# WanqingXia/UR-gym

Hardware: AMD Instinct MI355X
Metric: env-steps/sec (whole node) (higher is better)
Workload: dtype f64; 1 GPU; UR5DynReach-v1 N=65536 per GPU, random actions U(-1,1), auto-reset, seed 0; envs_total=65536, gather_obs=False, rollout_api=False, gjk_start=bullet

## Files before the change

ur_gym_amd/csrc/urgym_hip.hip:

```cpp
#include <hip/hip_runtime.h>
#include <stdint.h>
#include <stdio.h>
#include <string.h>
#include <math.h>
#include <new>
#include <vector>

#include "../../include/urgym.h"
#include "../../data/ur5e_model.h"
#include "urgym_device.h"
#include "urgym_launch_plan.h"
#include "urgym_actor.h"
#include "urgym_tables_host.h"

using namespace urgym;


namespace {

constexpr int WAVES = 4;
constexpr int THREADS = GROUP * WAVES;
constexpr uint32_t NO_ITEM = 0xFFFFFFFFu;
constexpr int REFILL_MIN = 16;
constexpr int RESIDENT = 3;
// ... 416 lines not shown
  int& s_left = L.s_left;
  auto& s_key = L.s_key;
  auto& s_pose = L.s_pose;

  const urgym_config& cfg = P.cfg;
  const urgym_buffers& B = P.buf;
  const int N = cfg.num_envs;
  const int tid = threadIdx.x;
  const int lane = tid & 63;
  const int wv = __builtin_amdgcn_readfirstlane(tid >> 6);
  constexpr int OD = (KIND == URGYM_ENV_ORI) ? 18 : ((KIND == URGYM_ENV_OBS) ? 26 : ((KIND == URGYM_ENV_STA) ? 29 : 35));
  constexpr int GD = (KIND == URGYM_ENV_OBS) ? 3 : 6;
  int vb = bidx;
  if (MODE == MODE_STEP && P.envs_tail == 0) {
    const int nb = nblk, x = vb & 7, per = nb >> 3, rem = nb & 7;
    vb = x * per + (x < rem ? x : rem) + (vb >> 3);
  }
  const bool tail_block = (MODE == MODE_STEP) && P.envs_tail > 0 && vb >= P.big_blocks;
  const int E = tail_block ? P.envs_tail : P.envs;
  const int first = tail_block ? P.big_blocks * P.envs + (vb - P.big_blocks) * P.envs_tail : vb * P.envs;
  const int G = (E + GROUP - 1) / GROUP;
  constexpr bool HAS_OBST = (KIND != URGYM_ENV_ORI);
  constexpr int COLL_BIT = 1 << 30;
  constexpr int EE_BIT = 1 << 29;
  constexpr int EPA_SHIFT = 8, EPA_MASK = 0x7FFF << EPA_SHIFT;
  const bool need_epa = WITH_EPA && ((KIND == URGYM_ENV_OBS) || !cfg.check_collision || (MODE != MODE_STEP));
  XRef pose_slot{(URGYM_LDS double*)&s_pose[0][0] + tid, THREADS};
  float* const s_out = reinterpret_cast<float*>(&s_pose[0][0]);
  static_assert(sizeof(float) * STEP_MAX_ENVS * 47 <= sizeof(double) * GJK_SLOT_DOUBLES * THREADS, "staging must fit");
  auto dist_cell = [&](int i, int e) -> double* {
    return DIST_LDS ? (double*)&s_dist[i][DIST_LDS ? e : 0] : &P.ld_scratch[(size_t)i * N + first + e];
  };

  if (bidx == 0 && tid == 0) {
    if (P.rzero) *P.rzero = 0;
    if (P.rzero2) *P.rzero2 = 0;
  }
  int list_count = 0;
  if (MODE != MODE_STEP) {
    list_count = (MODE == MODE_PREFETCH) ? min(*P.rcount, P.rcap) : B.done_count[P.pp];
    if (first >= list_count) return;
  }
  if (tid == 0) { s_ticket = THREADS; s_pending = 0; s_p1done = 0; s_left = 0; }
  if (MODE == MODE_STEP && tid < 8) {
    const int k = tid & 3, ex = tid >> 2;
    const bool tbl = (k == Q_TABLE);
    const double msum = M_HULL + ((k == 3) ? M_CYL : ((k == Q_SELF) ? M_HULL : (tbl ? M_TABLE : M_TRACK)));
// ... 85 lines not shown
      D3 a0[3], a1[3];
#pragma unroll
      for (int k = 0; k < 6; k++) {
        double sn, cs;
        if (use_cache) { sn = SOA(P.sc_scratch, 2 * k, n, N); cs = SOA(P.sc_scratch, 2 * k + 1, n, N); }
        else sincos(q[k], &sn, &cs);
        fk_joint(T, k, sn, cs);
        const int link = k + 1;
        const double* c = c_tab.capsule[k];
        const D3 b0 = apply(T, d3(c[0], c[1], c[2])), b1 = apply(T, d3(c[3], c[4], c[5]));
        const double rb = c[6];
        if (k < 3) { a0[k] = b0; a1[k] = b1; }
        if (link >= 2) {
          if (seg_box_lower_bound(b0, b1, TABLE_CX, TABLE_CY, TABLE_CZ, TABLE_HX, TABLE_HY, TABLE_HZ) - rb <= lim) pairs |= 1u << (PAIR_TABLE + link - 2);
          if (seg_box_lower_bound(b0, b1, TRACK_CX, TRACK_CY, TRACK_CZ, TRACK_HX, TRACK_HY, TRACK_HZ) - rb <= lim) pairs |= 1u << (PAIR_TRACK + link - 2);
        }
#pragma unroll
        for (int A = 1; A <= 3; A++) {
          if (A <= link - 2) {
            if (segseg_dist(a0[A - 1], a1[A - 1], b0, b1) - c_tab.capsule[A - 1][6] - rb <= lim + M_HULL) pairs |= 1u << self_pair_bit(A, link);
          }
        }
      }
      if (MODE == MODE_STEP) {
        double er, ep, ey;
        rpy_from_quat(rot_to_quat(T.r), er, ep, ey);
        float* orow = B.observation + (size_t)n * OD;
        orow[0] = (float)T.t.x; orow[1] = (float)T.t.y; orow[2] = (float)T.t.z;
        orow[3] = (float)er; orow[4] = (float)ep; orow[5] = (float)ey;
        atomicOr(&s_flags[e], EE_BIT);
      }
    }
    s_pairs[e] = pairs;
    if (pairs) atomicAdd(&s_pending, __popc(pairs));
  }
  if (MODE == MODE_STEP) {
    if (wv >= WAVES - G && lane == 0) __hip_atomic_fetch_add(&s_p1done, 1, __ATOMIC_RELEASE, __HIP_MEMORY_SCOPE_WORKGROUP);
  } else {
    __syncthreads();
  }

  if (!(MODE == MODE_STEP && !HAS_OBST && !cfg.check_collision)) {
    D3 v0 = d3(0, 1, 0);
    int kind = 3, e = 0, lb = 2, la = 1;
    auto shape_a = [&]() -> ShapeDesc { return hull_desc(kind == Q_SELF ? la : lb); };
    auto shape_b = [&]() -> ShapeDesc {
      ShapeDesc s;
      s.type = (kind == 3) ? SH_CYLZ : ((kind == Q_SELF) ? SH_HULL : SH_BOX);
      s.hull = lb - 1;
      const bool tbl = (kind == Q_TABLE);
      s.hx = (kind == 3) ? (CYL_R - M_CYL) : (tbl ? (TABLE_HX - M_TABLE) : (TRACK_HX - M_TRACK));
      s.hy = (kind == 3) ? (CYL_R - M_CYL) : (tbl ? (TABLE_HY - M_TABLE) : (TRACK_HY - M_TRACK));
      s.hz = (kind == 3) ? (0.5 * CYL_H - M_CYL) : (tbl ? (TABLE_HZ - M_TABLE) : (TRACK_HZ - M_TRACK));
      return s;
    };
    bool exact = false;
    const bool guided = cfg.gjk_start == URGYM_GJK_START_GUIDED;
    auto capsule_mid = [&](int link, const X3& TX) -> D3 {
      const double* c = c_tab.capsule[link - 1];
      return apply(TX, d3(0.5 * (c[0] + c[3]), 0.5 * (c[1] + c[4]), 0.5 * (c[2] + c[5])));
    };
    auto guided_axis = [&](D3 mid, D3 centre) -> D3 {
      const D3 d = mid - centre;
      const double n2 = dot(d, d);
      return n2 > 1e-12 ? d * (1.0 / sqrt(n2)) : d3(0, 1, 0);
// ... 126 lines not shown
      }
      typedef int pool_words __attribute__((ext_vector_type(4)));
      const pool_words pool = *(volatile URGYM_LDS pool_words*)(URGYM_LDS void*)&s_ticket;
      __builtin_amdgcn_fence(__ATOMIC_ACQUIRE, "workgroup");
      const bool more_tickets = pool.x < n_tickets;
      const bool p1_published = (MODE != MODE_STEP) || pool.z >= G;
      const bool more_pairs = pool.y > 0;
      if (MODE == MODE_STEP) p1_ok = p1_published;
      const int idle_lanes = __popcll(__ballot(!busy));
      if (!busy && (idle_lanes >= REFILL_MIN || idle_lanes == 64)) {
        uint32_t item = NO_ITEM;
        if (more_tickets) {
          const int t = atomicAdd(&s_ticket, 1);
          if (t < n_tickets) item = ticket_item(t);
        } else if (more_pairs) {
          if (atomicSub(&s_pending, 1) > 0) item = claim_pair();
        }
        if (item != NO_ITEM) {
          busy = setup(item);
          if (busy) gjk_begin(run, v0);
        }
      }
      if (__ballot(busy) == 0ull && !more_tickets && !more_pairs && p1_published) break;
    }
    auto epa_pass = [&]() -> bool {
      const EpaWs ws{(URGYM_LDS double*)&s_pose[0][0] + GROUP * wv, THREADS};
      bool armed = false;
#pragma unroll 1
      for (int g = 0; g < G; g++) {
        const int sl = g * GROUP + lane;
        const int marks = (sl < E) ? ((__hip_atomic_load(&s_flags[sl], __ATOMIC_RELAXED, __HIP_MEMORY_SCOPE_WORKGROUP) & EPA_MASK) >> EPA_SHIFT) : 0;
        unsigned long long envs_marked = __ballot(marks != 0);
#pragma unroll 1
        while (envs_marked) {
          const int el = __builtin_ctzll(envs_marked);
          envs_marked &= envs_marked - 1ull;
          const int ee = g * GROUP + el;
          int me = __shfl(marks, el);
#pragma unroll 1
          while (me) {
            const int b = __builtin_ctz((unsigned)me);
            me &= me - 1;
            int mine = 0;
            if (lane == 0) mine = (atomicAnd(&s_flags[ee], ~(1 << (EPA_SHIFT + b))) >> (EPA_SHIFT + b)) & 1;
            if (!__shfl(mine, 0)) continue;
            if (!armed) {
// ... 1 lines not shown
              if (MODE == MODE_STEP) p1_ok = true;
              armed = true;
            }
            const int body = b / 5, link = 2 + b - 5 * body;
            const uint32_t item = (uint32_t)ee | ((uint32_t)(body == 0 ? 3 : (body == 1 ? Q_TABLE : Q_TRACK)) << 8) | ((uint32_t)link << 10) |
                                  ((body ? 1u : 0u) << 16);
            if (!setup(item)) continue;
            epa_wave_sync();
            bool capped;
            const double depth = epa_wave(P.graph, shape_a(), shape_b(), ws, lane, capped);
            if (lane == 0) {
              const double dist = -(depth + margin_sum());
              if (workbench) atomicMin(reinterpret_cast<long long*>(dist_cell(lb - 2, e)), sortable(dist));
              else *dist_cell(lb - 2, e) = dist;
              if (capped) atomicOr(&s_flags[e], URGYM_STATUS_GJK_ITER);
            }
          }
        }
      }
      if (armed) pose_slot.p = (URGYM_LDS double*)&s_pose[0][0] + tid;
      return armed;
    };
    if (HAS_OBST && WITH_EPA) {
      if (lane == 0) __hip_atomic_fetch_add(&s_left, 1, __ATOMIC_RELEASE, __HIP_MEMORY_SCOPE_WORKGROUP);
#pragma unroll 1
      for (;;) {
        const int left = __hip_atomic_load(&s_left, __ATOMIC_ACQUIRE, __HIP_MEMORY_SCOPE_WORKGROUP);
        const bool served = epa_pass();
        if (!served && left >= WAVES) break;
        if (!served) __builtin_amdgcn_s_sleep(16);
      }
    }
    __syncthreads();
  }

  const int pe = (wv - (WAVES - G)) * GROUP + lane;
  if (wv >= WAVES - G && pe < E && s_env[pe] != -1) {
    const int n = s_env[pe] >= 0 ? s_env[pe] : -2 - s_env[pe];
    double q[6];
    for (int i = 0; i < 6; i++) q[i] = LDS_Q ? s_q[i][pe] : joint_of_step<MODE>(P, actions, n, i);
    const bool ee_ready = (MODE == MODE_STEP) && (s_flags[pe] & EE_BIT);
    X3 TE = identity_x3();
    if (!ee_ready) {
      if (KIND == URGYM_ENV_ORI) {
        double sn[6], cs[6];
#pragma unroll
        for (int k = 0; k < 6; k++) sincos(q[k], &sn[k], &cs[k]);
#pragma unroll
        for (int k = 0; k < 6; k++) fk_joint(TE, k, sn[k], cs[k]);
      } else {
#pragma unroll 1
        for (int k = 0; k < 6; k++) {
          double sn, cs;
          sincos(q[k], &sn, &cs);
          fk_joint(TE, k, sn, cs);
        }
      }
    }
    double opos[3] = {0, 0, 0};
    Q4 oq{0, 0, 0, 1};
    if (HAS_OBST) {
      if (LDS_STATE) {
        opos[0] = s_obst[0][pe]; opos[1] = s_obst[1][pe]; opos[2] = s_obst[2][pe];
        oq = Q4{s_obst[3][pe], s_obst[4][pe], s_obst[5][pe], s_obst[6][pe]};
      } else if (s_env[pe] >= 0) {
        for (int i = 0; i < 3; i++) opos[i] = SOA(P.sc_scratch, 12 + i, n, N);
        oq = Q4{SOA(P.sc_scratch, 15, n, N), SOA(P.sc_scratch, 16, n, N), SOA(P.sc_scratch, 17, n, N), SOA(P.sc_scratch, 18, n, N)};
      } else {
        obstacle_of_step<KIND>(P, n, opos, oq);
      }
    }
    const int step_count = B.step_count[n];
    float* row = &s_out[pe * 47];
    float ach[6];
    if (ee_ready) {
      for (int i = 0; i < 6; i++) ach[i] = B.observation[(size_t)n * OD + i];
    } else {
      Q4 eq = rot_to_quat(TE.r);
      double er, ep, ey;
      rpy_from_quat(eq, er, ep, ey);
      ach[0] = (float)TE.t.x; ach[1] = (float)TE.t.y; ach[2] = (float)TE.t.z;
      ach[3] = (float)er; ach[4] = (float)ep; ach[5] = (float)ey;
    }
    double goal[6];
    for (int i = 0; i < 6; i++) goal[i] = SOA(B.goal, i, n, N);
    double ld_old[5] = {0, 0, 0, 0, 0}, ld_new[5] = {0, 0, 0, 0, 0};
    bool coll = (s_flags[pe] & COLL_BIT) != 0;
    if (HAS_OBST) {
      for (int i = 0; i < 5; i++) {
        ld_new[i] = workbench ? unsortable(__double_as_longlong(*dist_cell(i, pe))) : *dist_cell(i, pe);
        if (MODE == MODE_STEP) ld_old[i] = SOA(B.link_dist, i, n, N);
        if (cfg.check_collision && ld_new[i] <= cfg.collision_margin) coll = true;
      }
    }
    if (MODE == MODE_PREFETCH) {
      const int key = s_key[pe], sl = key & 1;
      int rflags = s_flags[pe] & ~(COLL_BIT | EE_BIT | EPA_MASK);
      if (coll) rflags |= URGYM_STATUS_RESET_COLLISION;
      if (HAS_OBST) {
        for (int i = 0; i < 5; i++) REC(P, sl, REC_LD + i, n) = ld_new[i];
        REC(P, sl, REC_QUAT + 0, n) = oq.x; REC(P, sl, REC_QUAT + 1, n) = oq.y; REC(P, sl, REC_QUAT + 2, n) = oq.z; REC(P, sl, REC_QUAT + 3, n) = oq.w;
        double vel[6] = {0, 0, 0, 0, 0, 0};
        if (KIND == URGYM_ENV_DYN) {
          double st[6], en[6];
          for (int i = 0; i < 6; i++) { st[i] = REC(P, sl, REC_START + i, n); en[i] = REC(P, sl, REC_END + i, n); }
          dyn_velocity(st, en, cfg.dyn_time_duration, vel);
        }
        double dp[3];
        step_displacement(vel, cfg.dt, dp);
        for (int i = 0; i < 6; i++) REC(P, sl, REC_VEL + i, n) = vel[i];
        for (int i = 0; i < 3; i++) REC(P, sl, REC_DP + i, n) = dp[i];
      }
      RECI(P, sl, 1, n) = rflags;
      __threadfence();
      RECI(P, sl, 0, n) = key;
    }
    if (MODE != MODE_PREFETCH) {
    double vobs[6] = {0, 0, 0, 0, 0, 0};
    if (KIND == URGYM_ENV_DYN) {
      if (MODE == MODE_STEP) {
        if (step_count < cfg.dyn_motion_steps)
          for (int i = 0; i < 6; i++) vobs[i] = SOA(B.obst_vel, i, n, N);
      } else {
        for (int i = 0; i < 6; i++) vobs[i] = (double)B.observation[(size_t)n * OD + 24 + i];
      }
    }
    if (MODE == MODE_RESET && P.copy_final) {
      for (int i = 0; i < OD; i++) B.final_observation[(size_t)n * OD + i] = B.observation[(size_t)n * OD + i];
      for (int i = 0; i < GD; i++) {
        B.final_achieved_goal[(size_t)n * GD + i] = B.achieved_goal[(size_t)n * GD + i];
        B.final_desired_goal[(size_t)n * GD + i] = B.desired_goal[(size_t)n * GD + i];
      }
    }
    const double* ld_obs = (MODE == MODE_STEP) ? ld_old : ld_new;
    auto write_row = [&](const float* ach_, const double* q_, const double* goal_, const double* obst6_, const double* opos_, Q4 oq_,
                         const double* vobs_, const double* ld_) {
      int p = 0;
      for (int i = 0; i < 6; i++) row[p++] = ach_[i];
      for (int i = 0; i < 6; i++) row[p++] = (float)q_[i];
      if (KIND == URGYM_ENV_ORI) {
        for (int i = 0; i < 6; i++) row[p++] = (float)goal_[i];
      } else if (KIND == URGYM_ENV_OBS) {
        for (int i = 0; i < 3; i++) row[p++] = (float)goal_[i];
        for (int i = 0; i < 6; i++) row[p++] = (float)obst6_[i];
        for (int i = 0; i < 5; i++) row[p++] = (float)ld_[i];
      } else {
        for (int i = 0; i < 6; i++) row[p++] = (float)goal_[i];
        for (int i = 0; i < 3; i++) row[p++] = (float)opos_[i];
        double r_, p_, y_;
        rpy_from_quat(oq_, r_, p_, y_);
        row[p++] = (float)r_; row[p++] = (float)p_; row[p++] = (float)y_;
        if (KIND == URGYM_ENV_DYN)
          for (int i = 0; i < 6; i++) row[p++] = (float)vobs_[i];
        for (int i = 0; i < 5; i++) row[p++] = (float)ld_[i];
      }
      for (int i = 0; i < GD; i++) { row[OD + i] = ach_[i]; row[OD + GD + i] = (float)goal_[i]; }
    };
    double obst6[6] = {0, 0, 0, 0, 0, 0};
    if (KIND == URGYM_ENV_OBS)
      for (int i = 0; i < 6; i++) obst6[i] = SOA(B.obst_start, i, n, N);
    write_row(ach, q, goal, obst6, opos, oq, vobs, ld_obs);

    const double a6[6] = {(double)ach[0], (double)ach[1], (double)ach[2], (double)ach[3], (double)ach[4], (double)ach[5]};
    const double d = pos_distance(a6, goal);
    double th = 0.0;
    bool succ;
    if (KIND == URGYM_ENV_OBS) {
      succ = d < cfg.distance_threshold;
    } else {
      th = angular_distance(a6 + 3, goal + 3);
      succ = (d < cfg.distance_threshold) && (th < cfg.ori_threshold);
    }
    int flags = s_flags[pe] & ~(COLL_BIT | EE_BIT | EPA_MASK);
    if (MODE == MODE_STEP) {
      bool terminated = succ || coll;
      bool info_success = terminated ? !coll : false;
      double reward = 0.0;
      bool update_ld = false;
      if (KIND == URGYM_ENV_ORI) {
        reward += succ ? cfg.w_success : 0.0;
        reward += d * cfg.w_distance;
        reward += th * cfg.w_orientation;
        reward += coll ? cfg.w_collision : 0.0;
      } else if (KIND == URGYM_ENV_OBS) {
        reward += succ ? cfg.w_success : 0.0;
        reward += coll ? cfg.w_collision : 0.0;
        reward += cfg.w_distance * d;
        double sum = 0.0;
        for (int i = 0; i < 5; i++) sum += (ld_new[i] < cfg.near_threshold) ? cfg.w_link[i] * (ld_new[i] - ld_old[i]) : 0.0;
        reward += sum;
        update_ld = true;
      } else {
        if (coll) reward = cfg.w_collision;
        else if (succ) reward = cfg.w_success;
        else {
          reward += cfg.w_distance * d;
          reward += cfg.w_orientation * th;
          double sum = 0.0;
          for (int i = 0; i < 5; i++) sum += (ld_new[i] < cfg.near_threshold) ? cfg.w_link[i] * (ld_new[i] - ld_old[i]) : 0.0;
          reward += sum;
          update_ld = true;
        }
      }
      if (reward != reward) flags |= URGYM_STATUS_NAN;
      if (!update_ld) flags &= ~(URGYM_STATUS_PENETRATION | URGYM_STATUS_GJK_ITER);
      int sc = step_count + 1;
      bool truncated = sc >= cfg.max_episode_steps;
      for (int i = 0; i < 6; i++) SOA(B.q, i, n, N) = q[i];
      B.step_count[n] = sc;
      if (KIND == URGYM_ENV_DYN || KIND == URGYM_ENV_STA) {
        for (int i = 0; i < 3; i++) SOA(B.obst_pos, i, n, N) = opos[i];
        SOA(B.obst_quat, 0, n, N) = oq.x; SOA(B.obst_quat, 1, n, N) = oq.y; SOA(B.obst_quat, 2, n, N) = oq.z; SOA(B.obst_quat, 3, n, N) = oq.w;
      }
      if (update_ld)
        for (int i = 0; i < 5; i++) SOA(B.link_dist, i, n, N) = ld_new[i];
      B.reward[n] = (float)reward;
      B.terminated[n] = terminated ? 1 : 0;
      B.truncated[n] = truncated ? 1 : 0;
      B.is_success[n] = info_success ? 1 : 0;
      B.collision[n] = coll ? 1 : 0;
      if (cfg.auto_reset && (terminated || truncated)) {
        bool consumed = false;
        if (KIND == URGYM_ENV_ORI && P.inline_ori) {
          consumed = true;
          for (int i = 0; i < OD; i++) B.final_observation[(size_t)n * OD + i] = row[i];
          for (int i = 0; i < GD; i++) {
            B.final_achieved_goal[(size_t)n * GD + i] = row[OD + i];
            B.final_desired_goal[(size_t)n * GD + i] = row[OD + GD + i];
          }
          const int ecur = B.episode_id[n];
          double g2[6] = {0, 0, 0, 0, 0, 0}, none[6] = {0, 0, 0, 0, 0, 0}, q2[6], nold[5] = {0, 0, 0, 0, 0}, nop[3] = {0, 0, 0};
          sample_attempt<URGYM_ENV_ORI>(P, pose_slot, n, (uint32_t)ecur, 0, g2, none, none);
          for (int i = 0; i < 6; i++) { q2[i] = cfg.neutral_q[i]; SOA(B.goal, i, n, N) = g2[i]; SOA(B.q, i, n, N) = q2[i]; }
          B.step_count[n] = 0;
          B.episode_id[n] = ecur + 1;
          float ach2[6];
          for (int i = 0; i < 6; i++) ach2[i] = P.neutral_ach[i];
          write_row(ach2, q2, g2, none, nop, Q4{0, 0, 0, 1}, none, nold);
        } else if (P.prefetch) {
          const int ecur = B.episode_id[n], sl = ecur & 1;
          if (RECI(P, sl, 0, n) == ecur) {
            consumed = true;
            for (int i = 0; i < OD; i++) B.final_observation[(size_t)n * OD + i] = row[i];
            for (int i = 0; i < GD; i++) {
              B.final_achieved_goal[(size_t)n * GD + i] = row[OD + i];
              B.final_desired_goal[(size_t)n * GD + i] = row[OD + GD + i];
            }
            double g2[6], st2[6], ld2[5] = {0, 0, 0, 0, 0}, v2[6] = {0, 0, 0, 0, 0, 0}, q2[6], op2[3] = {0, 0, 0};
            Q4 oq2{0, 0, 0, 1};
            for (int i = 0; i < 6; i++) { g2[i] = REC(P, sl, REC_GOAL + i, n); st2[i] = REC(P, sl, REC_START + i, n); q2[i] = cfg.neutral_q[i]; }
            for (int i = 0; i < 6; i++) { SOA(B.goal, i, n, N) = g2[i]; SOA(B.q, i, n, N) = q2[i]; }
            if (HAS_OBST) {
              for (int i = 0; i < 6; i++) {
                SOA(B.obst_start, i, n, N) = st2[i];
                SOA(B.obst_end, i, n, N) = REC(P, sl, REC_END + i, n);
                SOA(B.obst_vel, i, n, N) = REC(P, sl, REC_VEL + i, n);
              }
              for (int i = 0; i < 3; i++) SOA(B.obst_vel, 6 + i, n, N) = REC(P, sl, REC_DP + i, n);
              oq2 = Q4{REC(P, sl, REC_QUAT + 0, n), REC(P, sl, REC_QUAT + 1, n), REC(P, sl, REC_QUAT + 2, n), REC(P, sl, REC_QUAT + 3, n)};
              for (int i = 0; i < 3; i++) { op2[i] = st2[i]; SOA(B.obst_pos, i, n, N) = st2[i]; }
              SOA(B.obst_quat, 0, n, N) = oq2.x; SOA(B.obst_quat, 1, n, N) = oq2.y; SOA(B.obst_quat, 2, n, N) = oq2.z; SOA(B.obst_quat, 3, n, N) = oq2.w;
              for (int i = 0; i < 5; i++) { ld2[i] = REC(P, sl, REC_LD + i, n); SOA(B.link_dist, i, n, N) = ld2[i]; }
              if (KIND == URGYM_ENV_DYN)
                for (int i = 0; i < 6; i++) v2[i] = (double)row[24 + i];
            }
            B.step_count[n] = 0;
            B.episode_id[n] = ecur + 1;
            flags |= RECI(P, sl, 1, n);
            float ach2[6];
            for (int i = 0; i < 6; i++) ach2[i] = P.neutral_ach[i];
            write_row(ach2, q2, g2, st2, op2, oq2, v2, ld2);
            const int pos = atomicAdd(P.rcount, 1);
            if (pos < P.rcap) P.rlist[pos] = make_int2(n, ecur + 2);
          }
        }
        if (!consumed) {
          int slot = atomicAdd(&B.done_count[P.pp], 1);
          B.done_list[slot] = n;
          if (P.prefetch && !P.fallback_on) atomicOr(&B.status[n], URGYM_STATUS_STALE_RECORD);
        }
      }
    } else {
      if (HAS_OBST) {
        for (int i = 0; i < 3; i++) SOA(B.obst_pos, i, n, N) = opos[i];
        SOA(B.obst_quat, 0, n, N) = oq.x; SOA(B.obst_quat, 1, n, N) = oq.y; SOA(B.obst_quat, 2, n, N) = oq.z; SOA(B.obst_quat, 3, n, N) = oq.w;
        for (int i = 0; i < 5; i++) SOA(B.link_dist, i, n, N) = ld_new[i];
        double vel[6] = {0, 0, 0, 0, 0, 0};
        if (KIND == URGYM_ENV_DYN) {
          double st[6], en[6];
          for (int i = 0; i < 6; i++) { st[i] = SOA(B.obst_start, i, n, N); en[i] = SOA(B.obst_end, i, n, N); }
          dyn_velocity(st, en, cfg.dyn_time_duration, vel);
        }
        double dp[3];
        step_displacement(vel, cfg.dt, dp);
        for (int i = 0; i < 6; i++) SOA(B.obst_vel, i, n, N) = vel[i];
        for (int i = 0; i < 3; i++) SOA(B.obst_vel, 6 + i, n, N) = dp[i];
      }
      if (MODE == MODE_RESET) {
        B.step_count[n] = 0;
        if (coll) flags |= URGYM_STATUS_RESET_COLLISION;
        if (P.prefetch) {
          const int k0 = s_key[pe];
          const int pos = atomicAdd(P.rcount, 2);
          if (pos + 1 < P.rcap) { P.rlist[pos] = make_int2(n, k0); P.rlist[pos + 1] = make_int2(n, k0 + 1); }
        }
        if (!P.copy_final) {
          B.reward[n] = 0.f; B.terminated[n] = 0; B.truncated[n] = 0;
          B.is_success[n] = succ ? 1 : 0;
          B.collision[n] = coll ? 1 : 0;
        }
      } else {
        B.is_success[n] = succ ? 1 : 0;
        B.collision[n] = coll ? 1 : 0;
      }
    }
    if (flags) atomicOr(&B.status[n], flags);
    }
  }
  __syncthreads();

  if (MODE == MODE_STEP) {
    const int base = first;
    const int cnt = min(E, N - base);
    for (int i = tid; i < cnt * OD; i += THREADS) __builtin_nontemporal_store(s_out[(i / OD) * 47 + (i % OD)], &B.observation[(size_t)base * OD + i]);
    for (int i = tid; i < cnt * GD; i += THREADS) {
      __builtin_nontemporal_store(s_out[(i / GD) * 47 + OD + (i % GD)], &B.achieved_goal[(size_t)base * GD + i]);
      __builtin_nontemporal_store(s_out[(i / GD) * 47 + OD + GD + (i % GD)], &B.desired_goal[(size_t)base * GD + i]);
    }
    if (bidx == 0 && tid == 0) B.done_count[P.pp ^ 1] = 0;
  } else if (MODE != MODE_PREFETCH) {
    const int cnt = min(E, list_count - first);
    for (int i = tid; i < cnt * OD; i += THREADS) {
      const int e = i / OD;
      const int se = s_env[e];
      const int ne = se >= 0 ? se : -2 - se;
      B.observation[(size_t)ne * OD + (i % OD)] = s_out[e * 47 + (i % OD)];
    }
    for (int i = tid; i < cnt * GD; i += THREADS) {
      const int e = i / GD;
      const int se = s_env[e];
      const int ne = se >= 0 ? se : -2 - se;
      B.achieved_goal[(size_t)ne * GD + (i % GD)] = s_out[e * 47 + OD + (i % GD)];
      B.desired_goal[(size_t)ne * GD + (i % GD)] = s_out[e * 47 + OD + GD + (i % GD)];
    }
  }
}

template <int KIND, int MODE, bool WITH_EPA>
__global__ void __launch_bounds__(THREADS, ((MODE == MODE_STEP || MODE == MODE_PREFETCH) ? RESIDENT : 2)) env_kernel(const KParams P, const float* __restrict__ actions) {
  __shared__ EnvLds<MODE> lds;
  env_body<KIND, MODE, WITH_EPA>(P, actions, lds, (int)blockIdx.x, (int)gridDim.x);
}
// ... 806 lines not shown
```

Baseline: 321.5 million env-steps/s.

## Split per-env finish into early/late phases run by waves leaving the GJK pool

Per-env finalisation is split into an early part (FK, achieved goal, observation row, success test) and a late part (collision, reward, state writes). In step mode, waves that leave the GJK work pool claim a finish rank and run the early part while other waves are still in EPA. Observation rows are then written straight to global memory instead of staged through LDS, which removes the final __syncthreads and the staging copy. In exchange, the global stores become scattered per-row writes rather than coalesced nontemporal stores, and the ordering between waves gets more complex.

```diff
diff --git a/ur_gym_amd/csrc/urgym_hip.hip b/ur_gym_amd/csrc/urgym_hip.hip
--- a/ur_gym_amd/csrc/urgym_hip.hip
+++ b/ur_gym_amd/csrc/urgym_hip.hip
@@ -462,7 +462,6 @@
   const int G = (E + GROUP - 1) / GROUP;
   constexpr bool HAS_OBST = (KIND != URGYM_ENV_ORI);
   constexpr int COLL_BIT = 1 << 30;
-  constexpr int EE_BIT = 1 << 29;
   constexpr int EPA_SHIFT = 8, EPA_MASK = 0x7FFF << EPA_SHIFT;
   const bool need_epa = WITH_EPA && ((KIND == URGYM_ENV_OBS) || !cfg.check_collision || (MODE != MODE_STEP));
   XRef pose_slot{(URGYM_LDS double*)&s_pose[0][0] + tid, THREADS};
@@ -594,14 +593,6 @@
           }
         }
       }
-      if (MODE == MODE_STEP) {
-        double er, ep, ey;
-        rpy_from_quat(rot_to_quat(T.r), er, ep, ey);
-        float* orow = B.observation + (size_t)n * OD;
-        orow[0] = (float)T.t.x; orow[1] = (float)T.t.y; orow[2] = (float)T.t.z;
-        orow[3] = (float)er; orow[4] = (float)ep; orow[5] = (float)ey;
-        atomicOr(&s_flags[e], EE_BIT);
-      }
     }
     s_pairs[e] = pairs;
     if (pairs) atomicAdd(&s_pending, __popc(pairs));
@@ -612,7 +603,320 @@
     __syncthreads();
   }
 
-  if (!(MODE == MODE_STEP && !HAS_OBST && !cfg.check_collision)) {
+  static_assert(WAVES > (STEP_MAX_ENVS + GROUP - 1) / GROUP, "the last wave to leave the pool must not be a finish wave");
+  const bool pooled = !(MODE == MODE_STEP && !HAS_OBST && !cfg.check_collision);
+  const bool direct = (MODE == MODE_STEP) && pooled;
+  const bool use_sc = (MODE == MODE_STEP) && (HAS_OBST || cfg.check_collision);
+  double f_q[6], f_opos[3], f_ld_old[5], f_d, f_th;
+  Q4 f_oq;
+  int f_sc;
+  bool f_succ;
+  auto row_ptrs = [&](int pe, int n, float*& orow, float*& arow, float*& drow) __attribute__((always_inline)) {
+    if (direct) {
+      orow = B.observation + (size_t)n * OD; arow = B.achieved_goal + (size_t)n * GD; drow = B.desired_goal + (size_t)n * GD;
+    } else {
+      orow = &s_out[pe * 47]; arow = orow + OD; drow = orow + OD + GD;
+    }
+  };
+  auto write_row = [&](float* orow, float* arow, float* drow, const float* ach_, const double* q_, const double* goal_, const double* obst6_,
+                       const double* opos_, Q4 oq_, const double* vobs_, const double* ld_) __attribute__((always_inline)) {
+    int p = 0;
+    for (int i = 0; i < 6; i++) orow[p++] = ach_[i];
+    for (int i = 0; i < 6; i++) orow[p++] = (float)q_[i];
+    if (KIND == URGYM_ENV_ORI) {
+      for (int i = 0; i < 6; i++) orow[p++] = (float)goal_[i];
+    } else if (KIND == URGYM_ENV_OBS) {
+      for (int i = 0; i < 3; i++) orow[p++] = (float)goal_[i];
+      for (int i = 0; i < 6; i++) orow[p++] = (float)obst6_[i];
+      for (int i = 0; i < 5; i++) orow[p++] = (float)ld_[i];
+    } else {
+      for (int i = 0; i < 6; i++) orow[p++] = (float)goal_[i];
+      for (int i = 0; i < 3; i++) orow[p++] = (float)opos_[i];
+      double r_, p_, y_;
+      rpy_from_quat(oq_, r_, p_, y_);
+      orow[p++] = (float)r_; orow[p++] = (float)p_; orow[p++] = (float)y_;
+      if (KIND == URGYM_ENV_DYN)
+        for (int i = 0; i < 6; i++) orow[p++] = (float)vobs_[i];
+      for (int i = 0; i < 5; i++) orow[p++] = (float)ld_[i];
+    }
+    for (int i = 0; i < GD; i++) { arow[i] = ach_[i]; drow[i] = (float)goal_[i]; }
+  };
+  auto finish_early = [&](const int pe) __attribute__((always_inline)) {
+    const int se = s_env[pe];
+    const int n = se >= 0 ? se : -2 - se;
+    for (int i = 0; i < 6; i++) f_q[i] = LDS_Q ? s_q[i][pe] : joint_of_step<MODE>(P, actions, n, i);
+    for (int i = 0; i < 3; i++) f_opos[i] = 0.0;
+    f_oq = Q4{0, 0, 0, 1};
+    if (HAS_OBST) {
+      if (LDS_STATE) {
+        f_opos[0] = s_obst[0][pe]; f_opos[1] = s_obst[1][pe]; f_opos[2] = s_obst[2][pe];
+        f_oq = Q4{s_obst[3][pe], s_obst[4][pe], s_obst[5][pe], s_obst[6][pe]};
+      } else if (se >= 0) {
+        for (int i = 0; i < 3; i++) f_opos[i] = SOA(P.sc_scratch, 12 + i, n, N);
+        f_oq = Q4{SOA(P.sc_scratch, 15, n, N), SOA(P.sc_scratch, 16, n, N), SOA(P.sc_scratch, 17, n, N), SOA(P.sc_scratch, 18, n, N)};
+      } else {
+        obstacle_of_step<KIND>(P, n, f_opos, f_oq);
+      }
+    }
+    if (MODE == MODE_PREFETCH) return;
+    f_sc = B.step_count[n];
+    const bool cached = use_sc && se >= 0;
+    X3 TE = identity_x3();
+    if (KIND == URGYM_ENV_ORI && !cached) {
+      double sn[6], cs[6];
+#pragma unroll
+      for (int k = 0; k < 6; k++) sincos(f_q[k], &sn[k], &cs[k]);
+#pragma unroll
+      for (int k = 0; k < 6; k++) fk_joint(TE, k, sn[k], cs[k]);
+    } else {
+#pragma unroll 1
+      for (int k = 0; k < 6; k++) {
+        double sn, cs;
+        if (cached) { sn = SOA(P.sc_scratch, 2 * k, n, N); cs = SOA(P.sc_scratch, 2 * k + 1, n, N); }
+        else sincos(LDS_Q ? s_q[k][pe] : joint_of_step<MODE>(P, actions, n, k), &sn, &cs);
+        fk_joint(TE, k, sn, cs);
+      }
+    }
+    float ach[6];
+    {
+      double er, ep, ey;
+      rpy_from_quat(rot_to_quat(TE.r), er, ep, ey);
+      ach[0] = (float)TE.t.x; ach[1] = (float)TE.t.y; ach[2] = (float)TE.t.z;
+      ach[3] = (float)er; ach[4] = (float)ep; ach[5] = (float)ey;
+    }
+    double goal[6];
+    for (int i = 0; i < 6; i++) goal[i] = SOA(B.goal, i, n, N);
+    double ld_row[5] = {0, 0, 0, 0, 0};
+    for (int i = 0; i < 5; i++) f_ld_old[i] = 0.0;
+    if (HAS_OBST) {
+      for (int i = 0; i < 5; i++) {
+        if (MODE == MODE_STEP) ld_row[i] = f_ld_old[i] = SOA(B.link_dist, i, n, N);
+        else ld_row[i] = workbench ? unsortable(__double_as_longlong(*dist_cell(i, pe))) : *dist_cell(i, pe);
+      }
+    }
+    double vobs[6] = {0, 0, 0, 0, 0, 0};
+    if (KIND == URGYM_ENV_DYN) {
+      if (MODE == MODE_STEP) {
+        if (f_sc < cfg.dyn_motion_steps)
+          for (int i = 0; i < 6; i++) vobs[i] = SOA(B.obst_vel, i, n, N);
+      } else {
+        for (int i = 0; i < 6; i++) vobs[i] = (double)B.observation[(size_t)n * OD + 24 + i];
+      }
+    }
+    if (MODE == MODE_RESET && P.copy_final) {
+      for (int i = 0; i < OD; i++) B.final_observation[(size_t)n * OD + i] = B.observation[(size_t)n * OD + i];
+      for (int i = 0; i < GD; i++) {
+        B.final_achieved_goal[(size_t)n * GD + i] = B.achieved_goal[(size_t)n * GD + i];
+        B.final_desired_goal[(size_t)n * GD + i] = B.desired_goal[(size_t)n * GD + i];
+      }
+    }
+    double obst6[6] = {0, 0, 0, 0, 0, 0};
+    if (KIND == URGYM_ENV_OBS)
+      for (int i = 0; i < 6; i++) obst6[i] = SOA(B.obst_start, i, n, N);
+    float *orow, *arow, *drow;
+    row_ptrs(pe, n, orow, arow, drow);
+    write_row(orow, arow, drow, ach, f_q, goal, obst6, f_opos, f_oq, vobs, ld_row);
+
+    const double a6[6] = {(double)ach[0], (double)ach[1], (double)ach[2], (double)ach[3], (double)ach[4], (double)ach[5]};
+    f_d = pos_distance(a6, goal);
+    f_th = 0.0;
+    if (KIND == URGYM_ENV_OBS) {
+      f_succ = f_d < cfg.distance_threshold;
+    } else {
+      f_th = angular_distance(a6 + 3, goal + 3);
+      f_succ = (f_d < cfg.distance_threshold) && (f_th < cfg.ori_threshold);
+    }
+    if (MODE == MODE_STEP) B.truncated[n] = (f_sc + 1 >= cfg.max_episode_steps) ? 1 : 0;
+  };
+  auto finish_late = [&](const int pe) __attribute__((always_inline)) {
+    const int se = s_env[pe];
+    const int n = se >= 0 ? se : -2 - se;
+    double ld_new[5] = {0, 0, 0, 0, 0};
+    bool coll = (s_flags[pe] & COLL_BIT) != 0;
+    if (HAS_OBST) {
+      for (int i = 0; i < 5; i++) {
+        ld_new[i] = workbench ? unsortable(__double_as_longlong(*dist_cell(i, pe))) : *dist_cell(i, pe);
+        if (cfg.check_collision && ld_new[i] <= cfg.collision_margin) coll = true;
+      }
+    }
+    if (MODE == MODE_PREFETCH) {
+      const int key = s_key[pe], sl = key & 1;
+      int rflags = s_flags[pe] & ~(COLL_BIT | EPA_MASK);
+      if (coll) rflags |= URGYM_STATUS_RESET_COLLISION;
+      if (HAS_OBST) {
+        for (int i = 0; i < 5; i++) REC(P, sl, REC_LD + i, n) = ld_new[i];
+        REC(P, sl, REC_QUAT + 0, n) = f_oq.x; REC(P, sl, REC_QUAT + 1, n) = f_oq.y; REC(P, sl, REC_QUAT + 2, n) = f_oq.z; REC(P, sl, REC_QUAT + 3, n) = f_oq.w;
+        double vel[6] = {0, 0, 0, 0, 0, 0};
+        if (KIND == URGYM_ENV_DYN) {
+          double st[6], en[6];
+          for (int i = 0; i < 6; i++) { st[i] = REC(P, sl, REC_START + i, n); en[i] = REC(P, sl, REC_END + i, n); }
+          dyn_velocity(st, en, cfg.dyn_time_duration, vel);
+        }
+        double dp[3];
+        step_displacement(vel, cfg.dt, dp);
+        for (int i = 0; i < 6; i++) REC(P, sl, REC_VEL + i, n) = vel[i];
+        for (int i = 0; i < 3; i++) REC(P, sl, REC_DP + i, n) = dp[i];
+      }
+      RECI(P, sl, 1, n) = rflags;
+      __threadfence();
+      RECI(P, sl, 0, n) = key;
+      return;
+    }
+    float *orow, *arow, *drow;
+    row_ptrs(pe, n, orow, arow, drow);
+    const double d = f_d, th = f_th;
+    const bool succ = f_succ;
+    int flags = s_flags[pe] & ~(COLL_BIT | EPA_MASK);
+    if (MODE == MODE_STEP) {
+      bool terminated = succ || coll;
+      bool info_success = terminated ? !coll : false;
+      double reward = 0.0;
+      bool update_ld = false;
+      if (KIND == URGYM_ENV_ORI) {
+        reward += succ ? cfg.w_success : 0.0;
+        reward += d * cfg.w_distance;
+        reward += th * cfg.w_orientation;
+        reward += coll ? cfg.w_collision : 0.0;
+      } else if (KIND == URGYM_ENV_OBS) {
+        reward += succ ? cfg.w_success : 0.0;
+        reward += coll ? cfg.w_collision : 0.0;
+        reward += cfg.w_distance * d;
+        double sum = 0.0;
+        for (int i = 0; i < 5; i++) sum += (ld_new[i] < cfg.near_threshold) ? cfg.w_link[i] * (ld_new[i] - f_ld_old[i]) : 0.0;
+        reward += sum;
+        update_ld = true;
+      } else {
+        if (coll) reward = cfg.w_collision;
+        else if (succ) reward = cfg.w_success;
+        else {
+          reward += cfg.w_distance * d;
+          reward += cfg.w_orientation * th;
+          double sum = 0.0;
+          for (int i = 0; i < 5; i++) sum += (ld_new[i] < cfg.near_threshold) ? cfg.w_link[i] * (ld_new[i] - f_ld_old[i]) : 0.0;
+          reward += sum;
+          update_ld = true;
+        }
+      }
+      if (reward != reward) flags |= URGYM_STATUS_NAN;
+      if (!update_ld) flags &= ~(URGYM_STATUS_PENETRATION | URGYM_STATUS_GJK_ITER);
+      const int sc = f_sc + 1;
+      const bool truncated = sc >= cfg.max_episode_steps;
+      for (int i = 0; i < 6; i++) SOA(B.q, i, n, N) = f_q[i];
+      B.step_count[n] = sc;
+      if (KIND == URGYM_ENV_DYN || KIND == URGYM_ENV_STA) {
+        for (int i = 0; i < 3; i++) SOA(B.obst_pos, i, n, N) = f_opos[i];
+        SOA(B.obst_quat, 0, n, N) = f_oq.x; SOA(B.obst_quat, 1, n, N) = f_oq.y; SOA(B.obst_quat, 2, n, N) = f_oq.z; SOA(B.obst_quat, 3, n, N) = f_oq.w;
+      }
+      if (update_ld)
+        for (int i = 0; i < 5; i++) SOA(B.link_dist, i, n, N) = ld_new[i];
+      B.reward[n] = (float)reward;
+      B.terminated[n] = terminated ? 1 : 0;
+      B.is_success[n] = info_success ? 1 : 0;
+      B.collision[n] = coll ? 1 : 0;
+      if (cfg.auto_reset && (terminated || truncated)) {
+        bool consumed = false;
+        if (KIND == URGYM_ENV_ORI && P.inline_ori) {
+          consumed = true;
+          for (int i = 0; i < OD; i++) B.final_observation[(size_t)n * OD + i] = orow[i];
+          for (int i = 0; i < GD; i++) {
+            B.final_achieved_goal[(size_t)n * GD + i] = arow[i];
+            B.final_desired_goal[(size_t)n * GD + i] = drow[i];
+          }
+          const int ecur = B.episode_id[n];
+          double g2[6] = {0, 0, 0, 0, 0, 0}, none[6] = {0, 0, 0, 0, 0, 0}, q2[6], nold[5] = {0, 0, 0, 0, 0}, nop[3] = {0, 0, 0};
+          sample_attempt<URGYM_ENV_ORI>(P, pose_slot, n, (uint32_t)ecur, 0, g2, none, none);
+          for (int i = 0; i < 6; i++) { q2[i] = cfg.neutral_q[i]; SOA(B.goal, i, n, N) = g2[i]; SOA(B.q, i, n, N) = q2[i]; }
+          B.step_count[n] = 0;
+          B.episode_id[n] = ecur + 1;
+          float ach2[6];
+          for (int i = 0; i < 6; i++) ach2[i] = P.neutral_ach[i];
+          write_row(orow, arow, drow, ach2, q2, g2, none, nop, Q4{0, 0, 0, 1}, none, nold);
+        } else if (P.prefetch) {
+          const int ecur = B.episode_id[n], sl = ecur & 1;
+          if (RECI(P, sl, 0, n) == ecur) {
+            consumed = true;
+            for (int i = 0; i < OD; i++) B.final_observation[(size_t)n * OD + i] = orow[i];
+            for (int i = 0; i < GD; i++) {
+              B.final_achieved_goal[(size_t)n * GD + i] = arow[i];
+              B.final_desired_goal[(size_t)n * GD + i] = drow[i];
+            }
+            double g2[6], st2[6], ld2[5] = {0, 0, 0, 0, 0}, v2[6] = {0, 0, 0, 0, 0, 0}, q2[6], op2[3] = {0, 0, 0};
+            Q4 oq2{0, 0, 0, 1};
+            for (int i = 0; i < 6; i++) { g2[i] = REC(P, sl, REC_GOAL + i, n); st2[i] = REC(P, sl, REC_START + i, n); q2[i] = cfg.neutral_q[i]; }
+            for (int i = 0; i < 6; i++) { SOA(B.goal, i, n, N) = g2[i]; SOA(B.q, i, n, N) = q2[i]; }
+            if (HAS_OBST) {
+              for (int i = 0; i < 6; i++) {
+                SOA(B.obst_start, i, n, N) = st2[i];
+                SOA(B.obst_end, i, n, N) = REC(P, sl, REC_END + i, n);
+                SOA(B.obst_vel, i, n, N) = REC(P, sl, REC_VEL + i, n);
+              }
+              for (int i = 0; i < 3; i++) SOA(B.obst_vel, 6 + i, n, N) = REC(P, sl, REC_DP + i, n);
+              oq2 = Q4{REC(P, sl, REC_QUAT + 0, n), REC(P, sl, REC_QUAT + 1, n), REC(P, sl, REC_QUAT + 2, n), REC(P, sl, REC_QUAT + 3, n)};
+              for (int i = 0; i < 3; i++) { op2[i] = st2[i]; SOA(B.obst_pos, i, n, N) = st2[i]; }
+              SOA(B.obst_quat, 0, n, N) = oq2.x; SOA(B.obst_quat, 1, n, N) = oq2.y; SOA(B.obst_quat, 2, n, N) = oq2.z; SOA(B.obst_quat, 3, n, N) = oq2.w;
+              for (int i = 0; i < 5; i++) { ld2[i] = REC(P, sl, REC_LD + i, n); SOA(B.link_dist, i, n, N) = ld2[i]; }
+              if (KIND == URGYM_ENV_DYN)
+                for (int i = 0; i < 6; i++) v2[i] = (double)orow[24 + i];
+            }
+            B.step_count[n] = 0;
+            B.episode_id[n] = ecur + 1;
+            flags |= RECI(P, sl, 1, n);
+            float ach2[6];
+            for (int i = 0; i < 6; i++) ach2[i] = P.neutral_ach[i];
+            write_row(orow, arow, drow, ach2, q2, g2, st2, op2, oq2, v2, ld2);
+            const int pos = atomicAdd(P.rcount, 1);
+            if (pos < P.rcap) P.rlist[pos] = make_int2(n, ecur + 2);
+          }
+        }
+        if (!consumed) {
+          int slot = atomicAdd(&B.done_count[P.pp], 1);
+          B.done_list[slot] = n;
+          if (P.prefetch && !P.fallback_on) atomicOr(&B.status[n], URGYM_STATUS_STALE_RECORD);
+        }
+      }
+    } else {
+      if (HAS_OBST) {
+        for (int i = 0; i < 3; i++) SOA(B.obst_pos, i, n, N) = f_opos[i];
+        SOA(B.obst_quat, 0, n, N) = f_oq.x; SOA(B.obst_quat, 1, n, N) = f_oq.y; SOA(B.obst_quat, 2, n, N) = f_oq.z; SOA(B.obst_quat, 3, n, N) = f_oq.w;
+        for (int i = 0; i < 5; i++) SOA(B.link_dist, i, n, N) = ld_new[i];
+        double vel[6] = {0, 0, 0, 0, 0, 0};
+        if (KIND == URGYM_ENV_DYN) {
+          double st[6], en[6];
+          for (int i = 0; i < 6; i++) { st[i] = SOA(B.obst_start, i, n, N); en[i] = SOA(B.obst_end, i, n, N); }
+          dyn_velocity(st, en, cfg.dyn_time_duration, vel);
+        }
+        double dp[3];
+        step_displacement(vel, cfg.dt, dp);
+        for (int i = 0; i < 6; i++) SOA(B.obst_vel, i, n, N) = vel[i];
+        for (int i = 0; i < 3; i++) SOA(B.obst_vel, 6 + i, n, N) = dp[i];
+      }
+      if (MODE == MODE_RESET) {
+        B.step_count[n] = 0;
+        if (coll) flags |= URGYM_STATUS_RESET_COLLISION;
+        if (P.prefetch) {
+          const int k0 = s_key[pe];
+          const int pos = atomicAdd(P.rcount, 2);
+          if (pos + 1 < P.rcap) { P.rlist[pos] = make_int2(n, k0); P.rlist[pos + 1] = make_int2(n, k0 + 1); }
+        }
+        if (!P.copy_final) {
+          B.reward[n] = 0.f; B.terminated[n] = 0; B.truncated[n] = 0;
+          B.is_success[n] = succ ? 1 : 0;
+          B.collision[n] = coll ? 1 : 0;
+        }
+      } else {
+        B.is_success[n] = succ ? 1 : 0;
+        B.collision[n] = coll ? 1 : 0;
+      }
+    }
+    if (flags) atomicOr(&B.status[n], flags);
+  };
+  int fin = -1;
+  auto finish_slot = [&]() -> int {
+    const int pe = fin * GROUP + lane;
+    return (fin >= 0 && pe < E && s_env[pe] != -1) ? pe : -1;
+  };
+
+  if (pooled) {
     D3 v0 = d3(0, 1, 0);
     int kind = 3, e = 0, lb = 2, la = 1;
     auto shape_a = [&]() -> ShapeDesc { return hull_desc(kind == Q_SELF ? la : lb); };
@@ -785,6 +1089,14 @@
         }
       }
       if (__ballot(busy) == 0ull && !more_tickets && !more_pairs && p1_published) break;
+    }
+    if (MODE == MODE_STEP) {
+      int rank = 0;
+      if (lane == 0) rank = __hip_atomic_fetch_add(&s_left, 1, __ATOMIC_RELEASE, __HIP_MEMORY_SCOPE_WORKGROUP);
+      rank = __builtin_amdgcn_readfirstlane(rank);
+      fin = rank < G ? rank : -1;
+      const int pe = finish_slot();
+      if (pe >= 0) finish_early(pe);
     }
     auto epa_pass = [&]() -> bool {
       const EpaWs ws{(URGYM_LDS double*)&s_pose[0][0] + GROUP * wv, THREADS};
@@ -832,7 +1144,7 @@
       return armed;
     };
     if (HAS_OBST && WITH_EPA) {
-      if (lane == 0) __hip_atomic_fetch_add(&s_left, 1, __ATOMIC_RELEASE, __HIP_MEMORY_SCOPE_WORKGROUP);
+      if (MODE != MODE_STEP && lane == 0) __hip_atomic_fetch_add(&s_left, 1, __ATOMIC_RELEASE, __HIP_MEMORY_SCOPE_WORKGROUP);
 #pragma unroll 1
       for (;;) {
         const int left = __hip_atomic_load(&s_left, __ATOMIC_ACQUIRE, __HIP_MEMORY_SCOPE_WORKGROUP);
@@ -844,289 +1156,17 @@
     __syncthreads();
   }
 
-  const int pe = (wv - (WAVES - G)) * GROUP + lane;
-  if (wv >= WAVES - G && pe < E && s_env[pe] != -1) {
-    const int n = s_env[pe] >= 0 ? s_env[pe] : -2 - s_env[pe];
-    double q[6];
-    for (int i = 0; i < 6; i++) q[i] = LDS_Q ? s_q[i][pe] : joint_of_step<MODE>(P, actions, n, i);
-    const bool ee_ready = (MODE == MODE_STEP) && (s_flags[pe] & EE_BIT);
-    X3 TE = identity_x3();
-    if (!ee_ready) {
-      if (KIND == URGYM_ENV_ORI) {
-        double sn[6], cs[6];
-#pragma unroll
-        for (int k = 0; k < 6; k++) sincos(q[k], &sn[k], &cs[k]);
-#pragma unroll
-        for (int k = 0; k < 6; k++) fk_joint(TE, k, sn[k], cs[k]);
-      } else {
-#pragma unroll 1
-        for (int k = 0; k < 6; k++) {
-          double sn, cs;
-          sincos(q[k], &sn, &cs);
-          fk_joint(TE, k, sn, cs);
-        }
-      }
-    }
-    double opos[3] = {0, 0, 0};
-    Q4 oq{0, 0, 0, 1};
-    if (HAS_OBST) {
-      if (LDS_STATE) {
-        opos[0] = s_obst[0][pe]; opos[1] = s_obst[1][pe]; opos[2] = s_obst[2][pe];
-        oq = Q4{s_obst[3][pe], s_obst[4][pe], s_obst[5][pe], s_obst[6][pe]};
-      } else if (s_env[pe] >= 0) {
-        for (int i = 0; i < 3; i++) opos[i] = SOA(P.sc_scratch, 12 + i, n, N);
-        oq = Q4{SOA(P.sc_scratch, 15, n, N), SOA(P.sc_scratch, 16, n, N), SOA(P.sc_scratch, 17, n, N), SOA(P.sc_scratch, 18, n, N)};
-      } else {
-        obstacle_of_step<KIND>(P, n, opos, oq);
-      }
-    }
-    const int step_count = B.step_count[n];
-    float* row = &s_out[pe * 47];
-    float ach[6];
-    if (ee_ready) {
-      for (int i = 0; i < 6; i++) ach[i] = B.observation[(size_t)n * OD + i];
-    } else {
-      Q4 eq = rot_to_quat(TE.r);
-      double er, ep, ey;
-      rpy_from_quat(eq, er, ep, ey);
-      ach[0] = (float)TE.t.x; ach[1] = (float)TE.t.y; ach[2] = (float)TE.t.z;
-      ach[3] = (float)er; ach[4] = (float)ep; ach[5] = (float)ey;
-    }
-    double goal[6];
-    for (int i = 0; i < 6; i++) goal[i] = SOA(B.goal, i, n, N);
-    double ld_old[5] = {0, 0, 0, 0, 0}, ld_new[5] = {0, 0, 0, 0, 0};
-    bool coll = (s_flags[pe] & COLL_BIT) != 0;
-    if (HAS_OBST) {
-      for (int i = 0; i < 5; i++) {
-        ld_new[i] = workbench ? unsortable(__double_as_longlong(*dist_cell(i, pe))) : *dist_cell(i, pe);
-        if (MODE == MODE_STEP) ld_old[i] = SOA(B.link_dist, i, n, N);
-        if (cfg.check_collision && ld_new[i] <= cfg.collision_margin) coll = true;
-      }
-    }
-    if (MODE == MODE_PREFETCH) {
-      const int key = s_key[pe], sl = key & 1;
-      int rflags = s_flags[pe] & ~(COLL_BIT | EE_BIT | EPA_MASK);
-      if (coll) rflags |= URGYM_STATUS_RESET_COLLISION;
-      if (HAS_OBST) {
-        for (int i = 0; i < 5; i++) REC(P, sl, REC_LD + i, n) = ld_new[i];
-        REC(P, sl, REC_QUAT + 0, n) = oq.x; REC(P, sl, REC_QUAT + 1, n) = oq.y; REC(P, sl, REC_QUAT + 2, n) = oq.z; REC(P, sl, REC_QUAT + 3, n) = oq.w;
-        double vel[6] = {0, 0, 0, 0, 0, 0};
-        if (KIND == URGYM_ENV_DYN) {
-          double st[6], en[6];
-          for (int i = 0; i < 6; i++) { st[i] = REC(P, sl, REC_START + i, n); en[i] = REC(P, sl, REC_END + i, n); }
-          dyn_velocity(st, en, cfg.dyn_time_duration, vel);
-        }
-        double dp[3];
-        step_displacement(vel, cfg.dt, dp);
-        for (int i = 0; i < 6; i++) REC(P, sl, REC_VEL + i, n) = vel[i];
-        for (int i = 0; i < 3; i++) REC(P, sl, REC_DP + i, n) = dp[i];
-      }
-      RECI(P, sl, 1, n) = rflags;
-      __threadfence();
-      RECI(P, sl, 0, n) = key;
-    }
-    if (MODE != MODE_PREFETCH) {
-    double vobs[6] = {0, 0, 0, 0, 0, 0};
-    if (KIND == URGYM_ENV_DYN) {
-      if (MODE == MODE_STEP) {
-        if (step_count < cfg.dyn_motion_steps)
-          for (int i = 0; i < 6; i++) vobs[i] = SOA(B.obst_vel, i, n, N);
-      } else {
-        for (int i = 0; i < 6; i++) vobs[i] = (double)B.observation[(size_t)n * OD + 24 + i];
-      }
-    }
-    if (MODE == MODE_RESET && P.copy_final) {
-      for (int i = 0; i < OD; i++) B.final_observation[(size_t)n * OD + i] = B.observation[(size_t)n * OD + i];
-      for (int i = 0; i < GD; i++) {
-        B.final_achieved_goal[(size_t)n * GD + i] = B.achieved_goal[(size_t)n * GD + i];
-        B.final_desired_goal[(size_t)n * GD + i] = B.desired_goal[(size_t)n * GD + i];
-      }
-    }
-    const double* ld_obs = (MODE == MODE_STEP) ? ld_old : ld_new;
-    auto write_row = [&](const float* ach_, const double* q_, const double* goal_, const double* obst6_, const double* opos_, Q4 oq_,
-                         const double* vobs_, const double* ld_) {
-      int p = 0;
-      for (int i = 0; i < 6; i++) row[p++] = ach_[i];
-      for (int i = 0; i < 6; i++) row[p++] = (float)q_[i];
-      if (KIND == URGYM_ENV_ORI) {
-        for (int i = 0; i < 6; i++) row[p++] = (float)goal_[i];
-      } else if (KIND == URGYM_ENV_OBS) {
-        for (int i = 0; i < 3; i++) row[p++] = (float)goal_[i];
-        for (int i = 0; i < 6; i++) row[p++] = (float)obst6_[i];
-        for (int i = 0; i < 5; i++) row[p++] = (float)ld_[i];
-      } else {
-        for (int i = 0; i < 6; i++) row[p++] = (float)goal_[i];
-        for (int i = 0; i < 3; i++) row[p++] = (float)opos_[i];
-        double r_, p_, y_;
-        rpy_from_quat(oq_, r_, p_, y_);
-        row[p++] = (float)r_; row[p++] = (float)p_; row[p++] = (float)y_;
-        if (KIND == URGYM_ENV_DYN)
-          for (int i = 0; i < 6; i++) row[p++] = (float)vobs_[i];
-        for (int i = 0; i < 5; i++) row[p++] = (float)ld_[i];
-      }
-      for (int i = 0; i < GD; i++) { row[OD + i] = ach_[i]; row[OD + GD + i] = (float)goal_[i]; }
-    };
-    double obst6[6] = {0, 0, 0, 0, 0, 0};
-    if (KIND == URGYM_ENV_OBS)
-      for (int i = 0; i < 6; i++) obst6[i] = SOA(B.obst_start, i, n, N);
-    write_row(ach, q, goal, obst6, opos, oq, vobs, ld_obs);
-
-    const double a6[6] = {(double)ach[0], (double)ach[1], (double)ach[2], (double)ach[3], (double)ach[4], (double)ach[5]};
-    const double d = pos_distance(a6, goal);
-    double th = 0.0;
-    bool succ;
-    if (KIND == URGYM_ENV_OBS) {
-      succ = d < cfg.distance_threshold;
-    } else {
-      th = angular_distance(a6 + 3, goal + 3);
-      succ = (d < cfg.distance_threshold) && (th < cfg.ori_threshold);
-    }
-    int flags = s_flags[pe] & ~(COLL_BIT | EE_BIT | EPA_MASK);
-    if (MODE == MODE_STEP) {
-      bool terminated = succ || coll;
-      bool info_success = terminated ? !coll : false;
-      double reward = 0.0;
-      bool update_ld = false;
-      if (KIND == URGYM_ENV_ORI) {
-        reward += succ ? cfg.w_success : 0.0;
-        reward += d * cfg.w_distance;
-        reward += th * cfg.w_orientation;
-        reward += coll ? cfg.w_collision : 0.0;
-      } else if (KIND == URGYM_ENV_OBS) {
-        reward += succ ? cfg.w_success : 0.0;
-        reward += coll ? cfg.w_collision : 0.0;
-        reward += cfg.w_distance * d;
-        double sum = 0.0;
-        for (int i = 0; i < 5; i++) sum += (ld_new[i] < cfg.near_threshold) ? cfg.w_link[i] * (ld_new[i] - ld_old[i]) : 0.0;
-        reward += sum;
-        update_ld = true;
-      } else {
-        if (coll) reward = cfg.w_collision;
-        else if (succ) reward = cfg.w_success;
-        else {
-          reward += cfg.w_distance * d;
-          reward += cfg.w_orientation * th;
-          double sum = 0.0;
-          for (int i = 0; i < 5; i++) sum += (ld_new[i] < cfg.near_threshold) ? cfg.w_link[i] * (ld_new[i] - ld_old[i]) : 0.0;
-          reward += sum;
-          update_ld = true;
-        }
-      }
-      if (reward != reward) flags |= URGYM_STATUS_NAN;
-      if (!update_ld) flags &= ~(URGYM_STATUS_PENETRATION | URGYM_STATUS_GJK_ITER);
-      int sc = step_count + 1;
-      bool truncated = sc >= cfg.max_episode_steps;
-      for (int i = 0; i < 6; i++) SOA(B.q, i, n, N) = q[i];
-      B.step_count[n] = sc;
-      if (KIND == URGYM_ENV_DYN || KIND == URGYM_ENV_STA) {
-        for (int i = 0; i < 3; i++) SOA(B.obst_pos, i, n, N) = opos[i];
-        SOA(B.obst_quat, 0, n, N) = oq.x; SOA(B.obst_quat, 1, n, N) = oq.y; SOA(B.obst_quat, 2, n, N) = oq.z; SOA(B.obst_quat, 3, n, N) = oq.w;
-      }
-      if (update_ld)
-        for (int i = 0; i < 5; i++) SOA(B.link_dist, i, n, N) = ld_new[i];
-      B.reward[n] = (float)reward;
-      B.terminated[n] = terminated ? 1 : 0;
-      B.truncated[n] = truncated ? 1 : 0;
-      B.is_success[n] = info_success ? 1 : 0;
-      B.collision[n] = coll ? 1 : 0;
-      if (cfg.auto_reset && (terminated || truncated)) {
-        bool consumed = false;
-        if (KIND == URGYM_ENV_ORI && P.inline_ori) {
-          consumed = true;
-          for (int i = 0; i < OD; i++) B.final_observation[(size_t)n * OD + i] = row[i];
-          for (int i = 0; i < GD; i++) {
-            B.final_achieved_goal[(size_t)n * GD + i] = row[OD + i];
-            B.final_desired_goal[(size_t)n * GD + i] = row[OD + GD + i];
-          }
-          const int ecur = B.episode_id[n];
-          double g2[6] = {0, 0, 0, 0, 0, 0}, none[6] = {0, 0, 0, 0, 0, 0}, q2[6], nold[5] = {0, 0, 0, 0, 0}, nop[3] = {0, 0, 0};
-          sample_attempt<URGYM_ENV_ORI>(P, pose_slot, n, (uint32_t)ecur, 0, g2, none, none);
-          for (int i = 0; i < 6; i++) { q2[i] = cfg.neutral_q[i]; SOA(B.goal, i, n, N) = g2[i]; SOA(B.q, i, n, N) = q2[i]; }
-          B.step_count[n] = 0;
-          B.episode_id[n] = ecur + 1;
-          float ach2[6];
-          for (int i = 0; i < 6; i++) ach2[i] = P.neutral_ach[i];
-          write_row(ach2, q2, g2, none, nop, Q4{0, 0, 0, 1}, none, nold);
-        } else if (P.prefetch) {
-          const int ecur = B.episode_id[n], sl = ecur & 1;
-          if (RECI(P, sl, 0, n) == ecur) {
-            consumed = true;
-            for (int i = 0; i < OD; i++) B.final_observation[(size_t)n * OD + i] = row[i];
-            for (int i = 0; i < GD; i++) {
-              B.final_achieved_goal[(size_t)n * GD + i] = row[OD + i];
-              B.final_desired_goal[(size_t)n * GD + i] = row[OD + GD + i];
-            }
-            double g2[6], st2[6], ld2[5] = {0, 0, 0, 0, 0}, v2[6] = {0, 0, 0, 0, 0, 0}, q2[6], op2[3] = {0, 0, 0};
-            Q4 oq2{0, 0, 0, 1};
-            for (int i = 0; i < 6; i++) { g2[i] = REC(P, sl, REC_GOAL + i, n); st2[i] = REC(P, sl, REC_START + i, n); q2[i] = cfg.neutral_q[i]; }
-            for (int i = 0; i < 6; i++) { SOA(B.goal, i, n, N) = g2[i]; SOA(B.q, i, n, N) = q2[i]; }
-            if (HAS_OBST) {
-              for (int i = 0; i < 6; i++) {
-                SOA(B.obst_start, i, n, N) = st2[i];
-                SOA(B.obst_end, i, n, N) = REC(P, sl, REC_END + i, n);
-                SOA(B.obst_vel, i, n, N) = REC(P, sl, REC_VEL + i, n);
-              }
-              for (int i = 0; i < 3; i++) SOA(B.obst_vel, 6 + i, n, N) = REC(P, sl, REC_DP + i, n);
-              oq2 = Q4{REC(P, sl, REC_QUAT + 0, n), REC(P, sl, REC_QUAT + 1, n), REC(P, sl, REC_QUAT + 2, n), REC(P, sl, REC_QUAT + 3, n)};
-              for (int i = 0; i < 3; i++) { op2[i] = st2[i]; SOA(B.obst_pos, i, n, N) = st2[i]; }
-              SOA(B.obst_quat, 0, n, N) = oq2.x; SOA(B.obst_quat, 1, n, N) = oq2.y; SOA(B.obst_quat, 2, n, N) = oq2.z; SOA(B.obst_quat, 3, n, N) = oq2.w;
-              for (int i = 0; i < 5; i++) { ld2[i] = REC(P, sl, REC_LD + i, n); SOA(B.link_dist, i, n, N) = ld2[i]; }
-              if (KIND == URGYM_ENV_DYN)
-                for (int i = 0; i < 6; i++) v2[i] = (double)row[24 + i];
-            }
-            B.step_count[n] = 0;
-            B.episode_id[n] = ecur + 1;
-            flags |= RECI(P, sl, 1, n);
-            float ach2[6];
-            for (int i = 0; i < 6; i++) ach2[i] = P.neutral_ach[i];
-            write_row(ach2, q2, g2, st2, op2, oq2, v2, ld2);
-            const int pos = atomicAdd(P.rcount, 1);
-            if (pos < P.rcap) P.rlist[pos] = make_int2(n, ecur + 2);
-          }
-        }
-        if (!consumed) {
-          int slot = atomicAdd(&B.done_count[P.pp], 1);
-          B.done_list[slot] = n;
-          if (P.prefetch && !P.fallback_on) atomicOr(&B.status[n], URGYM_STATUS_STALE_RECORD);
-        }
-      }
-    } else {
-      if (HAS_OBST) {
-        for (int i = 0; i < 3; i++) SOA(B.obst_pos, i, n, N) = opos[i];
-        SOA(B.obst_quat, 0, n, N) = oq.x; SOA(B.obst_quat, 1, n, N) = oq.y; SOA(B.obst_quat, 2, n, N) = oq.z; SOA(B.obst_quat, 3, n, N) = oq.w;
-        for (int i = 0; i < 5; i++) SOA(B.link_dist, i, n, N) = ld_new[i];
-        double vel[6] = {0, 0, 0, 0, 0, 0};
-        if (KIND == URGYM_ENV_DYN) {
-          double st[6], en[6];
-          for (int i = 0; i < 6; i++) { st[i] = SOA(B.obst_start, i, n, N); en[i] = SOA(B.obst_end, i, n, N); }
-          dyn_velocity(st, en, cfg.dyn_time_duration, vel);
-        }
-        double dp[3];
-        step_displacement(vel, cfg.dt, dp);
-        for (int i = 0; i < 6; i++) SOA(B.obst_vel, i, n, N) = vel[i];
-        for (int i = 0; i < 3; i++) SOA(B.obst_vel, 6 + i, n, N) = dp[i];
-      }
-      if (MODE == MODE_RESET) {
-        B.step_count[n] = 0;
-        if (coll) flags |= URGYM_STATUS_RESET_COLLISION;
-        if (P.prefetch) {
-          const int k0 = s_key[pe];
-          const int pos = atomicAdd(P.rcount, 2);
-          if (pos + 1 < P.rcap) { P.rlist[pos] = make_int2(n, k0); P.rlist[pos + 1] = make_int2(n, k0 + 1); }
-        }
-        if (!P.copy_final) {
-          B.reward[n] = 0.f; B.terminated[n] = 0; B.truncated[n] = 0;
-          B.is_success[n] = succ ? 1 : 0;
-          B.collision[n] = coll ? 1 : 0;
-        }
-      } else {
-        B.is_success[n] = succ ? 1 : 0;
-        B.collision[n] = coll ? 1 : 0;
-      }
-    }
-    if (flags) atomicOr(&B.status[n], flags);
-    }
-  }
+  if (!direct) {
+    fin = (wv >= WAVES - G) ? wv - (WAVES - G) : -1;
+    const int pe = finish_slot();
+    if (pe >= 0) finish_early(pe);
+  }
+  {
+    const int pe = finish_slot();
+    if (pe >= 0) finish_late(pe);
+  }
+  if (MODE == MODE_STEP && bidx == 0 && tid == 0) B.done_count[P.pp ^ 1] = 0;
+  if (direct) return;
   __syncthreads();
 
   if (MODE == MODE_STEP) {
@@ -1137,7 +1177,6 @@
       __builtin_nontemporal_store(s_out[(i / GD) * 47 + OD + (i % GD)], &B.achieved_goal[(size_t)base * GD + i]);
       __builtin_nontemporal_store(s_out[(i / GD) * 47 + OD + GD + (i % GD)], &B.desired_goal[(size_t)base * GD + i]);
     }
-    if (bidx == 0 && tid == 0) B.done_count[P.pp ^ 1] = 0;
   } else if (MODE != MODE_PREFETCH) {
     const int cnt = min(E, list_count - first);
     for (int i = tid; i < cnt * OD; i += THREADS) {
```

Result: no change. 323.5 million env-steps/s (median of 6 runs) (+0.6%).
